# Rita-zi/WavTokenizer

Hardware: AMD Instinct MI355X
Metric: audio-seconds/sec encode+decode, 24 kHz 3 s clips (higher is better)
Workload: dtype f32 (split-f16 x3 products)

## Files before the change

### wavtokenizer_amd/csrc/gemm.hip

```cpp
#include "common.h"
#include <stdlib.h>
#include <cmath>

namespace wt {

typedef float f32x4 __attribute__((ext_vector_type(4)));
typedef float f32x16 __attribute__((ext_vector_type(16)));

static constexpr int BK = 32;
static constexpr int LDS_PITCH = 36;

__device__ __forceinline__ int xcd_remap(int orig, int nwg) {
    int q = nwg >> 3, r = nwg & 7;
    int xcd = orig & 7, idx = orig >> 3;
    int base = xcd < r ? xcd * (q + 1) : r * (q + 1) + (xcd - r) * q;
    return base + idx;
}

__device__ __forceinline__ float elu1(float x) { return x > 0.f ? x : __expf(x) - 1.f; }
__device__ __forceinline__ float gelu_erf(float x) { return x * 0.5f * (1.f + erff(x * 0.70710678118654752440f)); }

template <int BM, int BN, int WAVES_M, int WAVES_N, int PRO, int EPI>
__global__ __launch_bounds__(256) void gemm_kernel(const GemmArgs p) {
    constexpr int WM = BM / WAVES_M, WN = BN / WAVES_N;
// ... 208 lines not shown
                const float bme = in ? p.bias[pc] : 0.f;
                const int f = (pc >> 5) * 16 + (col_l & 15);
#pragma unroll
                for (int r = 0; r < 16; ++r) {
                    const int m = m_w + i * 32 + (r & 3) + 8 * (r >> 2) + row_h;
                    const float mine = acc[i][j][r] + bme;
                    const float ph = __shfl_xor(mine, 16, 64);
                    if (is_mag && in && m < p.M) {
                        float mag = expf(mine);
                        mag = fminf(mag, 100.f);
                        Cg[(long)m * p.c_rstride + f] = mag * cosf(ph);
                        Cg[(long)m * p.c_rstride + p.head_kb + f] = mag * sinf(ph);
                    }
                }
            }
        return;
    }

#pragma unroll
    for (int i = 0; i < TM; ++i)
#pragma unroll
        for (int j = 0; j < TN; ++j) {
            const int n = n_w + j * 32 + col_l;
            if (n >= p.N) continue;
            float bn_ = 0.f, gm = 1.f;
            if (EPI == EPI_BIAS || EPI == EPI_BIAS_RES || EPI == EPI_BIAS_GELU || EPI == EPI_BIAS_GAMMA_RES ||
                EPI == EPI_BIAS_RES_ELU)
                bn_ = p.bias ? p.bias[n] : 0.f;
            if (EPI == EPI_BIAS_GAMMA_RES) gm = p.gamma[n];
#pragma unroll
            for (int r = 0; r < 16; ++r) {
                const int m = m_w + i * 32 + (r & 3) + 8 * (r >> 2) + row_h;
                if (m >= p.M) continue;
                float v = acc[i][j][r];
                if (EPI == EPI_BIAS) {
                    Cg[(long)m * p.c_rstride + n] = v + bn_;
                } else if (EPI == EPI_BIAS_RES) {
                    Cg[(long)m * p.c_rstride + n] = (v + bn_) + p.R[(long)m * p.r_rstride + n];
                } else if (EPI == EPI_BIAS_RES_ELU) {
                    Cg[(long)m * p.c_rstride + n] = elu1((v + bn_) + p.R[(long)m * p.r_rstride + n]);
                } else if (EPI == EPI_BIAS_GELU) {
                    Cg[(long)m * p.c_rstride + n] = gelu_erf(v + bn_);
                } else if (EPI == EPI_BIAS_GAMMA_RES) {
                    Cg[(long)m * p.c_rstride + n] = p.R[(long)m * p.r_rstride + n] + gm * (v + bn_);
                } else if (EPI == EPI_SCALE) {
                    Cg[(long)m * p.c_rstride + n] = v * p.alpha;
                } else if (EPI == EPI_BIAS_ROW) {
// ... 127 lines not shown
```

### wavtokenizer_amd/csrc/gemm16s_kernel.inc

```
template <int BM, int BN, int WAVES_M, int WAVES_N, int NSTAGE, int EPI, int OUT, int DBG = 0, int MF = WT_GEMM16S_MF, int WPS = 2, int KS = 1,
          int PROD = 0>
__global__ __launch_bounds__(64 * WAVES_M * WAVES_N * (1 + PROD), WPS) void G16_NAME(const GemmArgs p G16_PARAMS) {
    constexpr int dbg = DBG;
    static_assert(KS == 1 || (KS == 2 && NSTAGE == 6 && MF == 1 && DBG == 0), "two K tiles per barrier: 6 stages (three pairs), 16x16x32 MFMA, no experiment masks");
    static_assert(!PROD || KS == 2, "loader waves: the two-tiles-per-barrier form only");
    constexpr int NW = WAVES_M * WAVES_N, NT = 64 * NW * (1 + PROD);
    constexpr int NL = PROD ? NW * PROD : NW;
    constexpr int WM = BM / WAVES_M, WN = BN / WAVES_N;
    constexpr int TM = WM / 32, TN = WN / 32;
    constexpr int STG = (BM + BN) * 128;
    constexpr int NPA = BM / 8 / NL, NPB = BN / 8 / NL;
    constexpr int NPT = NPA + NPB;
    static_assert(BM % (8 * NL) == 0 && BN % (8 * NL) == 0, "pieces must divide evenly among the loading waves");
    static_assert(WM % 32 == 0 && WN % 32 == 0 && BM % 16 == 0, "32x32 MFMA tiles");
    static_assert((NSTAGE - 2) * NPT < 64, "vmcnt field");
    extern __shared__ __attribute__((aligned(1024))) char smem_s[];

    const int tid = threadIdx.x, lane = tid & 63;
    const int wave_all = (dbg & 65536) ? (tid >> 6) : __builtin_amdgcn_readfirstlane(tid >> 6);
    const bool loader_wave = PROD && wave_all >= NW;
    const bool mfma_wave = !loader_wave;
    const bool dma_wave = !PROD || loader_wave;
    const int wave = loader_wave ? wave_all - NW : wave_all;
    const int wm = wave / WAVES_N, wn = wave % WAVES_N;
// ... 612 lines not shown
                        }
#pragma unroll
                        for (int it = 0; it < 4; ++it) {
                            const int r = 8 * it + (lane >> 3), ch = lane & 7;
                            const int m = m_w + i * 32 + r;
                            const int n = n0 + 4 * ch;
                            if (m < p.M && (!as_f32 || n < p.N) && !(dbg & 128)) {
                                float* dst = dbase + (long)m * p.c_rstride + n;
                                store_c16<!(dbg & 4096)>(dst, q[it]);
                            }
                        }
                    }
                }
            }
        } else
#pragma unroll
        for (int i = 0; i < TM; ++i) {
#pragma unroll
            for (int j = 0; j < TN; ++j)
#pragma unroll
                for (int g = 0; g < 4; ++g) {
                    const int m = m_w + i * 32 + sub_row(g);
                    const int n = n_w + j * 32 + sub_col(g);
                    if (m >= p.M || n >= p.N) continue;
                    float* crow = Cg + (long)m * p.c_rstride;
                    f32x4 v = acc4(i, j, g);
                    if (EPI == EPI_SCALE || EPI == EPI_BIAS_ROW) {
                        v = EPI == EPI_SCALE ? v * p.alpha : v + p.bias[m];
                        if (n + 3 >= p.N) { if (n + 1 >= p.N) v.y = 0.f; if (n + 2 >= p.N) v.z = 0.f; v.w = 0.f; }
                    }
                    else if (p.bias) v += PCACHE ? *reinterpret_cast<const f32x4*>(pcw + (n - n_w) * 4) : *reinterpret_cast<const f32x4*>(p.bias + n);
                    if (EPI == EPI_BIAS_RES) {
                        v = v + *reinterpret_cast<const f32x4*>(p.R + (long)m * p.r_rstride + n);
                    } else if (EPI == EPI_BIAS_RES_ELU) {
                        v = v + *reinterpret_cast<const f32x4*>(p.R + (long)m * p.r_rstride + n);
                        v.x = elu_s(v.x); v.y = elu_s(v.y); v.z = elu_s(v.z); v.w = elu_s(v.w);
                    } else if (EPI == EPI_BIAS_ELU) {
                        v.x = elu_s(v.x); v.y = elu_s(v.y); v.z = elu_s(v.z); v.w = elu_s(v.w);
                    } else if (EPI == EPI_BIAS_GELU) {
                        v = (dbg & 16384) ? gelu_erf_s4(v) : gelu_erfc_s4(v);
                    } else if (EPI == EPI_BIAS_GAMMA_RES) {
                        const f32x4 gm = *reinterpret_cast<const f32x4*>(pcw + WN * 4 + (n - n_w) * 4);
                        v = *reinterpret_cast<const f32x4*>(p.R + (long)m * p.r_rstride + n) + gm * v;
                    }
                    if (OUT == OUT_S32 || OUT == OUT_S32_DUAL_ELU) store_s32_x4(crow, n, v, amax);
                    else store_c16<(dbg & 262144) != 0>(crow + n, v);
                    if (OUT == OUT_S32_DUAL_ELU) {
// ... 24 lines not shown
```

### wavtokenizer_amd/csrc/ops.hip

```cpp
#include "common.h"
#include <stdlib.h>

namespace wt {

typedef float f32x4 __attribute__((ext_vector_type(4)));

static inline void note_form(int kernel, int variant, int variant2, dim3 grid, unsigned block, size_t lds = 0) {
    if (OpForm* f = g_launch.form) *f = OpForm{kernel, variant, variant2, {grid.x, grid.y, grid.z}, block, (unsigned)lds};
}

__device__ __forceinline__ float wave_sum(float v) {
#pragma unroll
    for (int off = 32; off >= 1; off >>= 1) v += __shfl_xor(v, off, 64);
    return v;
}
typedef _Float16 f16x4s __attribute__((ext_vector_type(4)));
__device__ __forceinline__ void store_s32_1(float* row_base, int e, float v, float& amax) {
    amax = amax1(amax, v);
    _Float16* p = reinterpret_cast<_Float16*>(row_base) + ((e >> 5) * 64 + (e & 31));
    const _Float16 h = (_Float16)v;
    p[0] = h;
    p[32] = (_Float16)((v - (float)h) * 2048.f);
}
__device__ __forceinline__ void store_s32_4(float* row_base, int e, const f32x4 v, float& amax) {
    amax = amax4(amax, v.x, v.y, v.z, v.w);
    f16x4s hi, lo;
    split4_f16(v.x, v.y, v.z, v.w, hi, lo);
    _Float16* p = reinterpret_cast<_Float16*>(row_base) + ((e >> 5) * 64 + (e & 31));
    *reinterpret_cast<f16x4s*>(p) = hi;
    *reinterpret_cast<f16x4s*>(p + 32) = lo;
}
__device__ __forceinline__ float wave_max(float v) {
#pragma unroll
    for (int off = 32; off >= 1; off >>= 1) v = fmaxf(v, __shfl_xor(v, off, 64));
    return v;
}
__device__ __forceinline__ int reflect_pos(int pos, int T, int Tp, bool& ok) {
    if (pos < 0) pos = -pos;
    if (pos >= Tp) pos = 2 * (Tp - 1) - pos;
    ok = pos < T;
    return pos;
}

__global__ __launch_bounds__(256) void conv_first_kernel(const float* __restrict__ wav, const float* __restrict__ w,
                                                         const float* __restrict__ bias, float* __restrict__ y,
                                                         long BT, int T, int k, int Cout, int Tp) {
    const int c4n = Cout >> 2;
    const long total = BT * c4n;
    const int pl = (k - 1) - (k - 1) / 2;
    for (long idx = (long)blockIdx.x * blockDim.x + threadIdx.x; idx < total; idx += (long)gridDim.x * blockDim.x) {
        const long m = idx / c4n;
        const int c = (int)(idx - m * c4n) * 4;
        const long b = m / T;
// ... 110 lines not shown
    const int pl = (k - 1) - (k - 1) / 2, pr = (k - 1) / 2;
    const int maxpad = pl > pr ? pl : pr;
    const int Tp = T > maxpad ? (int)T : maxpad + 1;
    if (Cin == 32 && k == 7 && B <= 65535) {
        note_form(OPK_CONV_LAST32, 0, 0, dim3((unsigned)((T + 255) / 256), B), 256);
        hipLaunchKernelGGL(conv_last32_kernel, dim3((unsigned)((T + 255) / 256), B), dim3(256), 0, s, x, w, bias, y, (int)T, Tp, elu_in);
        WT_HIP_CHECK(hipGetLastError());
        return 0;
    }
    if (Cin < 4 || Cin > 256 || (Cin & (Cin - 1))) { set_error("conv_last: Cin must be a power of two in [4, 256]"); return -1; }
    const long groups = (BT + (256 / (Cin / 4)) - 1) / (256 / (Cin / 4));
    int blocks = (int)(groups < 16384 ? groups : 16384);
    note_form(OPK_CONV_LAST, 0, 0, dim3(blocks), 256);
    hipLaunchKernelGGL(conv_last_kernel, dim3(blocks), dim3(256), 0, s, x, w, bias, y, BT, (int)T, Cin, k, Tp, elu_in);
    WT_HIP_CHECK(hipGetLastError());
    return 0;
}

static constexpr int GN_CH = 128;
__device__ __forceinline__ int mix_len(const int* __restrict__ lens, int b, int Lpad) {
    const int l = lens[b];
    return l < 0 ? 0 : (l > Lpad ? Lpad : l);
}
#define OPS_MIX 0
#define OPS_K(base) base##_kernel
#define OPS_L L
#include "ops_kernel.inc"
#undef OPS_MIX
#undef OPS_K
#undef OPS_L
#define OPS_MIX 1
#define OPS_K(base) base##_mixed_kernel
#define OPS_L Lpad
#include "ops_kernel.inc"
#undef OPS_MIX
#undef OPS_K
#undef OPS_L

int launch_transpose(const float* in, float* out, int B, int R, int C, hipStream_t s, int out_s32, const int* lens) {
    if (out_s32 && (R % 32)) { set_error("transpose: an S32 output needs rows in multiples of 32 elements"); return -1; }
    dim3 grid((C + 31) / 32, (R + 31) / 32, B);
    if (lens) {
        note_form(OPK_TRANSPOSE_MIXED, 0, 0, grid, 256);
        hipLaunchKernelGGL(transpose_mixed_kernel, grid, dim3(256), 0, s, in, out, R, C, out_s32, g_launch.status, lens);
        WT_HIP_CHECK(hipGetLastError());
        return 0;
// ... 37 lines not shown
    const size_t smem = (size_t)GN_CH * GB * cg * sizeof(float);
    if (lens) {
        static PerDeviceOnce attr_mixed;
        if (int rc = attr_mixed.run([&]() -> int { WT_HIP_CHECK(hipFuncSetAttribute(reinterpret_cast<const void*>(gn_chunk_stats_mixed_kernel), hipFuncAttributeMaxDynamicSharedMemorySize, 64 * 1024)); return 0; })) return rc;
        hipLaunchKernelGGL(gn_chunk_stats_mixed_kernel, dim3(groups / GB, nch, B), dim3(256), smem, s, x, part, L, C, cg, GB, groups, nch, lens, lmin);
        const dim3 grid(groups / GB, mode ? nch : 1, B);
        if (mode == 0) hipLaunchKernelGGL(gn_chunk_apply_mixed_kernel<0>, grid, dim3(256), 0, s, x, part, gamma, beta, scale, shift, y, L, C, cg, GB, groups, nch, eps, out_s32, g_launch.status, lens, lmin);
        else if (mode == 1) hipLaunchKernelGGL(gn_chunk_apply_mixed_kernel<1>, grid, dim3(256), 0, s, x, part, gamma, beta, scale, shift, y, L, C, cg, GB, groups, nch, eps, out_s32, g_launch.status, lens, lmin);
        else hipLaunchKernelGGL(gn_chunk_apply_mixed_kernel<2>, grid, dim3(256), 0, s, x, part, gamma, beta, scale, shift, y, L, C, cg, GB, groups, nch, eps, out_s32, g_launch.status, lens, lmin);
        WT_HIP_CHECK(hipGetLastError());
        return 0;
    }
    static PerDeviceOnce attr_once;
    if (int rc = attr_once.run([&]() -> int { WT_HIP_CHECK(hipFuncSetAttribute(reinterpret_cast<const void*>(gn_chunk_stats_kernel), hipFuncAttributeMaxDynamicSharedMemorySize, 64 * 1024)); return 0; })) return rc;
    hipLaunchKernelGGL(gn_chunk_stats_kernel, dim3(groups / GB, nch, B), dim3(256), smem, s, x, part, L, C, cg, GB, groups, nch);
    const dim3 grid(groups / GB, mode ? nch : 1, B);
    note_form(OPK_GN_CHUNK, mode, 0, grid, 256, smem);
    if (mode == 0) hipLaunchKernelGGL(gn_chunk_apply_kernel<0>, grid, dim3(256), 0, s, x, part, gamma, beta, scale, shift, y, L, C, cg, GB, groups, nch, eps, out_s32, g_launch.status);
    else if (mode == 1) hipLaunchKernelGGL(gn_chunk_apply_kernel<1>, grid, dim3(256), 0, s, x, part, gamma, beta, scale, shift, y, L, C, cg, GB, groups, nch, eps, out_s32, g_launch.status);
    else hipLaunchKernelGGL(gn_chunk_apply_kernel<2>, grid, dim3(256), 0, s, x, part, gamma, beta, scale, shift, y, L, C, cg, GB, groups, nch, eps, out_s32, g_launch.status);
    WT_HIP_CHECK(hipGetLastError());
    return 0;
}
static int gn_slab_groups(int C, int groups) {
    const int cg = C / groups;
    for (int g = 1; g <= groups; ++g)
        if (groups % g == 0 && (g * cg) % 32 == 0 && g * cg <= 128) return g;
    return 0;
}

int launch_gn_apply(const float* x, const float* gamma, const float* beta, float* scale, float* shift, float* y,
                    int swish, int B, int L, int C, int groups, float eps, hipStream_t s, int out_s32, float* part, const int* lens) {
    if (out_s32 && (C % 32)) { set_error("gn_apply: an S32 output needs C % 32 == 0"); return -1; }
    const int cg = C / groups;
    int GB = 0;
    for (int g = 1; g <= groups; ++g)
        if (groups % g == 0 && (g * cg) % 32 == 0 && g * cg <= 128) { GB = g; break; }
    if (lens) {
        if (!GB || (cg % 4) || (C % 4) || GB > 8) { set_error("gn_apply: no length-aware form for this channel layout"); return -1; }
        const int lmax = (int)((96 * 1024) / ((size_t)GB * cg * 4));
        if (L > lmax && !part) { set_error("gn_apply: the length-aware launch needs the chunk scratch beyond the slab limit"); return -1; }
        const size_t smem = (size_t)(L < lmax ? L : lmax) * GB * cg * sizeof(float);
        static PerDeviceOnce attr_mixed;
        if (int rc = attr_mixed.run([&]() -> int {
            WT_HIP_CHECK(hipFuncSetAttribute(reinterpret_cast<const void*>(gn_tile_mixed_kernel<0>), hipFuncAttributeMaxDynamicSharedMemorySize, 96 * 1024));
            WT_HIP_CHECK(hipFuncSetAttribute(reinterpret_cast<const void*>(gn_tile_mixed_kernel<1>), hipFuncAttributeMaxDynamicSharedMemorySize, 96 * 1024));
            return 0;
        })) return rc;
        dim3 grid(groups / GB, B);
        const int nt = GB == 4 ? 512 : 256;
        note_form(OPK_GN_MIXED, swish ? 2 : 1, L > lmax ? 3 : 1, grid, nt, smem);
        if (swish) hipLaunchKernelGGL(gn_tile_mixed_kernel<1>, grid, dim3(nt), smem, s, x, gamma, beta, scale, shift, y, L, C, cg, GB, eps, out_s32, g_launch.status, lens, lmax);
        else hipLaunchKernelGGL(gn_tile_mixed_kernel<0>, grid, dim3(nt), smem, s, x, gamma, beta, scale, shift, y, L, C, cg, GB, eps, out_s32, g_launch.status, lens, lmax);
        WT_HIP_CHECK(hipGetLastError());
        if (L > lmax) return launch_gn_chunked(x, gamma, beta, scale, shift, y, swish ? 2 : 1, B, L, C, groups, GB, eps, s, out_s32, part, lens, lmax);
        return 0;
    }
    if (GB && (cg % 4 == 0) && (size_t)L * GB * cg * 4 <= 96 * 1024 && (C % 4 == 0)) {
        const size_t smem = (size_t)L * GB * cg * sizeof(float);
        static PerDeviceOnce attr_once;
        if (int rc = attr_once.run([&]() -> int {
            WT_HIP_CHECK(hipFuncSetAttribute(reinterpret_cast<const void*>(gn_tile_kernel<0>), hipFuncAttributeMaxDynamicSharedMemorySize, 96 * 1024));
            WT_HIP_CHECK(hipFuncSetAttribute(reinterpret_cast<const void*>(gn_tile_kernel<1>), hipFuncAttributeMaxDynamicSharedMemorySize, 96 * 1024));
        return 0;
    })) return rc;
        dim3 grid(groups / GB, B);
        const int nt = GB == 4 ? 512 : 256;
        note_form(OPK_GN_TILE, swish ? 1 : 0, (nt >> 6) == 2 * GB ? 2 : 1, grid, nt, smem);
        if (swish) hipLaunchKernelGGL(gn_tile_kernel<1>, grid, dim3(nt), smem, s, x, gamma, beta, scale, shift, y, L, C, cg, GB, eps, out_s32, g_launch.status);
        else hipLaunchKernelGGL(gn_tile_kernel<0>, grid, dim3(nt), smem, s, x, gamma, beta, scale, shift, y, L, C, cg, GB, eps, out_s32, g_launch.status);
        WT_HIP_CHECK(hipGetLastError());
        return 0;
    }
    if (part && GB && (cg % 4 == 0) && (C % 4 == 0) && GB * cg <= 128 && GB <= 8)
        return launch_gn_chunked(x, gamma, beta, scale, shift, y, swish ? 2 : 1, B, L, C, groups, GB, eps, s, out_s32, part);
    note_form(OPK_GN_STATS, swish ? 2 : 1, 0, dim3(groups, B), 256);
    if (swish)
        hipLaunchKernelGGL(gn_stats_kernel<2>, dim3(groups, B), dim3(256), 0, s, x, gamma, beta, scale, shift, y, L, C,
                           C / groups, eps, out_s32, g_launch.status);
    else
        hipLaunchKernelGGL(gn_stats_kernel<1>, dim3(groups, B), dim3(256), 0, s, x, gamma, beta, scale, shift, y, L, C,
                           C / groups, eps, out_s32, g_launch.status);
    WT_HIP_CHECK(hipGetLastError());
    return 0;
}

template <int NV, int MODE>
__global__ __launch_bounds__(256) void rownorm_kernel(const float* __restrict__ x, float* __restrict__ y, long M, int L,
                                                      const float* __restrict__ dw_w, const float* __restrict__ dw_b,
                                                      const float* __restrict__ in_scale,
                                                      const float* __restrict__ in_shift,
                                                      const float* __restrict__ out_scale,
                                                      const float* __restrict__ out_shift, float eps, int s32, unsigned* status) {
// ... 33 lines not shown
    float sum = 0.f;
#pragma unroll
    for (int i = 0; i < NV; ++i) sum += (v[i].x + v[i].y) + (v[i].z + v[i].w);
    const float mean = wave_sum(sum) * (1.f / C);
    float sq = 0.f;
#pragma unroll
    for (int i = 0; i < NV; ++i) {
        const f32x4 d = v[i] - mean;
        sq += (d.x * d.x + d.y * d.y) + (d.z * d.z + d.w * d.w);
    }
    const float rstd = 1.f / sqrtf(wave_sum(sq) * (1.f / C) + eps);
#pragma unroll
    for (int i = 0; i < NV; ++i) {
        const int c = (i * 64 + lane) * 4;
        const f32x4 os = *reinterpret_cast<const f32x4*>(out_scale + c);
        const f32x4 oh = *reinterpret_cast<const f32x4*>(out_shift + c);
        const f32x4 o = ((v[i] - mean) * rstd) * os + oh;
        if (s32) store_s32_4(y + m * C, c, o, amax);
        else *reinterpret_cast<f32x4*>(y + m * C + c) = o;
    }
    range_report(status, amax);
}

template <int NV>
static int launch_rownorm_nv(int mode, const float* x, float* y, long M, int L, const float* dw_w, const float* dw_b,
                             const float* is, const float* ih, const float* os, const float* oh, float eps,
                             hipStream_t s, int s32, const int* lens) {
    dim3 grid((unsigned)((M + 3) / 4));
    if (mode == RN_DWCONV && lens) {
        const int B = (int)(M / L);
        if (M <= 2048) {
            const long waves = (long)B * L;
            note_form(OPK_DWCONV_LN_MIXED, NV, 1, dim3((unsigned)((waves + 3) / 4)), 256);
            hipLaunchKernelGGL((dwconv_ln_mixed_kernel<NV, 1>), dim3((unsigned)((waves + 3) / 4)), dim3(256), 0, s, x, y, B, L, dw_w, dw_b,
                               os, oh, eps, s32, g_launch.status, lens);
        } else {
            constexpr int R = 4;
            const long waves = (long)B * ((L + R - 1) / R);
            note_form(OPK_DWCONV_LN_MIXED, NV, R, dim3((unsigned)((waves + 3) / 4)), 256);
            hipLaunchKernelGGL((dwconv_ln_mixed_kernel<NV, R>), dim3((unsigned)((waves + 3) / 4)), dim3(256), 0, s, x, y, B, L, dw_w, dw_b,
                               os, oh, eps, s32, g_launch.status, lens);
        }
    }
    else if (mode == RN_DWCONV) {
        const int B = (int)(M / L);
        if (M <= 2048) {
            const long waves = (long)B * L;
            note_form(OPK_DWCONV_LN, NV, 1, dim3((unsigned)((waves + 3) / 4)), 256);
            hipLaunchKernelGGL((dwconv_ln_kernel<NV, 1>), dim3((unsigned)((waves + 3) / 4)), dim3(256), 0, s, x, y, B, L, dw_w, dw_b,
                               os, oh, eps, s32, g_launch.status);
        } else {
            constexpr int R = 4;
            const long waves = (long)B * ((L + R - 1) / R);
            note_form(OPK_DWCONV_LN, NV, R, dim3((unsigned)((waves + 3) / 4)), 256);
            hipLaunchKernelGGL((dwconv_ln_kernel<NV, R>), dim3((unsigned)((waves + 3) / 4)), dim3(256), 0, s, x, y, B, L, dw_w, dw_b,
                               os, oh, eps, s32, g_launch.status);
        }
    }
    else if (mode == RN_PLAIN) {
        note_form(OPK_ROWNORM, NV, RN_PLAIN, grid, 256);
        hipLaunchKernelGGL((rownorm_kernel<NV, RN_PLAIN>), grid, dim3(256), 0, s, x, y, M, L, dw_w, dw_b, is, ih, os, oh, eps, s32, g_launch.status);
    } else {
        note_form(OPK_ROWNORM, NV, RN_AFFINE_IN, grid, 256);
        hipLaunchKernelGGL((rownorm_kernel<NV, RN_AFFINE_IN>), grid, dim3(256), 0, s, x, y, M, L, dw_w, dw_b, is, ih, os, oh, eps, s32, g_launch.status);
    }
    WT_HIP_CHECK(hipGetLastError());
    return 0;
}

int launch_rownorm(int mode, const float* x, float* y, int B, int L, int C, const float* dw_w, const float* dw_b,
                   const float* in_scale, const float* in_shift, const float* out_scale, const float* out_shift,
                   float eps, hipStream_t s, int out_s32, const int* lens) {
    const long M = (long)B * L;
    switch (C) {
        case 256: return launch_rownorm_nv<1>(mode, x, y, M, L, dw_w, dw_b, in_scale, in_shift, out_scale, out_shift, eps, s, out_s32, lens);
        case 512: return launch_rownorm_nv<2>(mode, x, y, M, L, dw_w, dw_b, in_scale, in_shift, out_scale, out_shift, eps, s, out_s32, lens);
        case 768: return launch_rownorm_nv<3>(mode, x, y, M, L, dw_w, dw_b, in_scale, in_shift, out_scale, out_shift, eps, s, out_s32, lens);
        case 1024: return launch_rownorm_nv<4>(mode, x, y, M, L, dw_w, dw_b, in_scale, in_shift, out_scale, out_shift, eps, s, out_s32, lens);
        default: set_error("rownorm: backbone dim must be 256, 512, 768 or 1024"); return -1;
    }
// ... 466 lines not shown
```

### wavtokenizer_amd/csrc/ops_kernel.inc

```

__global__ __launch_bounds__(256) void OPS_K(transpose)(const float* __restrict__ in, float* __restrict__ out, int R,
                                                        int C, int s32, unsigned* status
#if OPS_MIX
                                                        , const int* __restrict__ lens
#endif
                                                        ) {
    __shared__ float tile[32][33];
    float amax = 0.f;
    const long boff = (long)blockIdx.z * R * C;
    const int c0 = blockIdx.x * 32, r0 = blockIdx.y * 32;
    const int tx = threadIdx.x & 31, ty = threadIdx.x >> 5;
    for (int i = ty; i < 32; i += 8) {
        const int r = r0 + i, c = c0 + tx;
        if (r < R && c < C) tile[i][tx] = in[boff + (long)r * C + c];
    }
    __syncthreads();
    for (int i = ty; i < 32; i += 8) {
        const int c = c0 + i, r = r0 + tx;
        if (r < R && c < C) {
#if OPS_MIX
            const float v = c < mix_len(lens, blockIdx.z, C) ? tile[tx][i] : 0.f;
            if (s32) store_s32_1(out + boff + (long)c * R, r, v, amax);
            else out[boff + (long)c * R + r] = v;
#else
// ... 49 lines not shown
    if (threadIdx.x == 0) s_rstd = 1.f / sqrtf((red[0] + red[1] + red[2] + red[3]) / (float)n + eps);
    __syncthreads();
    if (threadIdx.x < cg) {
        const int c = g * cg + threadIdx.x;
        const float sc = s_rstd * gamma[c];
        scale[(long)b * C + c] = sc;
        shift[(long)b * C + c] = beta[c] - mean * sc;
    }
    if (APPLY) {
        float* yb = y + (long)b * OPS_L * C + g * cg;
        const float rstd = s_rstd;
        for (int i = threadIdx.x; i < n; i += 256) {
            const int t = i / cg, j = i - t * cg;
            const float sc = rstd * gamma[g * cg + j];
            float v = xb[(long)t * C + j] * sc + (beta[g * cg + j] - mean * sc);
            if (APPLY == 2) v = v / (1.f + expf(-v));
            if (s32) store_s32_1(y + ((long)b * OPS_L + t) * C, g * cg + j, v, amax);
            else yb[(long)t * C + j] = v;
        }
        range_report(status, amax);
    }
}

template <int SWISH>
__global__ __launch_bounds__(512) void OPS_K(gn_tile)(const float* __restrict__ x, const float* __restrict__ gamma,
                                                      const float* __restrict__ beta, float* __restrict__ scale,
                                                      float* __restrict__ shift, float* __restrict__ y, int OPS_L, int C,
                                                      int cg, int GB, float eps, int s32, unsigned* status
#if OPS_MIX
                                                      , const int* __restrict__ lens, int lmax
#endif
                                                      ) {
    extern __shared__ __attribute__((aligned(16))) float tile[];
    float amax = 0.f;
    __shared__ float s_sc[128], s_sh[128], s_red[8];
    const int NT = blockDim.x;
    const int W = GB * cg, W4 = W / 4;
    const int c0 = blockIdx.x * W, b = blockIdx.y;
#if OPS_MIX
    const int L = mix_len(lens, b, Lpad);
    if (L > lmax) return;
#endif
    const float* xb = x + (long)b * OPS_L * C + c0;
    const int dt = NT / W4, dq = NT - dt * W4;
    {
        int t = threadIdx.x / W4, q = threadIdx.x - t * W4;
        for (; t < L; t += dt, q += dq) {
// ... 65 lines not shown
        }
    }
    __syncthreads();
    float* yb = y + (long)b * OPS_L * C;
#if OPS_MIX
    for (int e = threadIdx.x; e < (Lpad - L) * W4; e += NT) {
        const int tz = e / W4, q = e - tz * W4;
        const f32x4 z = {0.f, 0.f, 0.f, 0.f};
        if (s32) store_s32_4(yb + (long)(L + tz) * C, c0 + q * 4, z, amax);
        else *reinterpret_cast<f32x4*>(yb + (long)(L + tz) * C + c0 + q * 4) = z;
    }
#endif
    {
        int t = threadIdx.x / W4, q = threadIdx.x - t * W4;
        for (; t < L; t += dt, q += dq) {
            if (q >= W4) { q -= W4; ++t; if (t >= L) break; }
            const f32x4 v = *reinterpret_cast<const f32x4*>(tile + t * W + q * 4);
            const f32x4 sc = *reinterpret_cast<const f32x4*>(s_sc + q * 4), sh = *reinterpret_cast<const f32x4*>(s_sh + q * 4);
            f32x4 o = v * sc + sh;
            if (SWISH) {
                o.x *= __builtin_amdgcn_rcpf(1.f + __expf(-o.x)); o.y *= __builtin_amdgcn_rcpf(1.f + __expf(-o.y));
                o.z *= __builtin_amdgcn_rcpf(1.f + __expf(-o.z)); o.w *= __builtin_amdgcn_rcpf(1.f + __expf(-o.w));
            }
            if (s32) store_s32_4(yb + (long)t * C, c0 + q * 4, o, amax);
            else *reinterpret_cast<f32x4*>(yb + (long)t * C + c0 + q * 4) = o;
        }
    }
    range_report(status, amax);
}


__global__ __launch_bounds__(256) void OPS_K(gn_chunk_stats)(const float* __restrict__ x, float* __restrict__ part, int OPS_L,
                                                             int C, int cg, int GB, int groups, int nch
#if OPS_MIX
                                                             , const int* __restrict__ lens, int lmin
#endif
                                                             ) {
    extern __shared__ __attribute__((aligned(16))) float tile[];
    const int W = GB * cg, W4 = W / 4;
    const int c0 = blockIdx.x * W, k = blockIdx.y, b = blockIdx.z;
#if OPS_MIX
    const int L = mix_len(lens, b, Lpad);
    if (L <= lmin || k * GN_CH >= L) return;
#endif
    const int t0 = k * GN_CH, rows = L - t0 < GN_CH ? L - t0 : GN_CH;
    const float* xb = x + ((long)b * OPS_L + t0) * C + c0;
    for (int e = threadIdx.x; e < rows * W4; e += 256) {
        const int t = e / W4, q = e - t * W4;
// ... 80 lines not shown
        f32x4 o = v * sc + sh;
        if (APPLY == 2) {
            o.x *= __builtin_amdgcn_rcpf(1.f + __expf(-o.x)); o.y *= __builtin_amdgcn_rcpf(1.f + __expf(-o.y));
            o.z *= __builtin_amdgcn_rcpf(1.f + __expf(-o.z)); o.w *= __builtin_amdgcn_rcpf(1.f + __expf(-o.w));
        }
        if (s32) store_s32_4(yb + (long)t * C, c0 + q * 4, o, amax);
        else *reinterpret_cast<f32x4*>(yb + (long)t * C + c0 + q * 4) = o;
    }
#if OPS_MIX
    {
        const int rz0 = rows > 0 ? rows : 0, rz1 = Lpad - t0 < GN_CH ? Lpad - t0 : GN_CH;
        const f32x4 z = {0.f, 0.f, 0.f, 0.f};
        for (int e = threadIdx.x + rz0 * W4; e < rz1 * W4; e += 256) {
            const int t = e / W4, q = e - t * W4;
            if (s32) store_s32_4(yb + (long)t * C, c0 + q * 4, z, amax);
            else *reinterpret_cast<f32x4*>(yb + (long)t * C + c0 + q * 4) = z;
        }
    }
#endif
#undef OPS_NCH
    range_report(status, amax);
}

template <int NV, int R>
__global__ __launch_bounds__(256) void OPS_K(dwconv_ln)(const float* __restrict__ x, float* __restrict__ y, int B, int OPS_L,
                                                        const float* __restrict__ dw_w, const float* __restrict__ dw_b,
                                                        const float* __restrict__ out_scale,
                                                        const float* __restrict__ out_shift, float eps, int s32, unsigned* status
#if OPS_MIX
                                                        , const int* __restrict__ lens
#endif
                                                        ) {
    constexpr int C = NV * 256;
    const int lane = threadIdx.x & 63;
    float amax = 0.f;
    const int per_clip = (OPS_L + R - 1) / R;
    const long wq = (long)blockIdx.x * 4 + (threadIdx.x >> 6);
    if (wq >= (long)B * per_clip) return;
    const int b = (int)(wq / per_clip);
    const int t0 = (int)(wq - (long)b * per_clip) * R;
#if OPS_MIX
    const int L = mix_len(lens, b, Lpad);
#endif
    const float* xb = x + (long)b * OPS_L * C;
    f32x4 v[R][NV];
#pragma unroll
    for (int i = 0; i < NV; ++i) {
        const int c = (i * 64 + lane) * 4;
        f32x4 xr[R + 6], w[7];
#pragma unroll
        for (int k = 0; k < R + 6; ++k) {
            const int tt = t0 + k - 3;
            xr[k] = (tt >= 0 && tt < L) ? *reinterpret_cast<const f32x4*>(xb + (long)tt * C + c) : (f32x4){0.f, 0.f, 0.f, 0.f};
        }
#pragma unroll
        for (int j = 0; j < 7; ++j) w[j] = *reinterpret_cast<const f32x4*>(dw_w + j * C + c);
        const f32x4 bias = *reinterpret_cast<const f32x4*>(dw_b + c);
#pragma unroll
        for (int r = 0; r < R; ++r) {
            f32x4 acc = bias;
#pragma unroll
            for (int j = 0; j < 7; ++j) {
                const int tt = t0 + r + j - 3;
                if (tt >= 0 && tt < L) acc += xr[r + j] * w[j];
            }
            v[r][i] = acc;
        }
    }
#pragma unroll
    for (int r = 0; r < R; ++r) {
#if OPS_MIX
        if (t0 + r >= Lpad) break;
        if (t0 + r >= L) {
            float* zrow = y + ((long)b * Lpad + t0 + r) * C;
            const f32x4 z = {0.f, 0.f, 0.f, 0.f};
#pragma unroll
            for (int i = 0; i < NV; ++i) {
                const int c = (i * 64 + lane) * 4;
                if (s32) store_s32_4(zrow, c, z, amax);
                else *reinterpret_cast<f32x4*>(zrow + c) = z;
            }
            continue;
        }
#else
        if (t0 + r >= L) break;
#endif
        float sum = 0.f;
#pragma unroll
        for (int i = 0; i < NV; ++i) sum += (v[r][i].x + v[r][i].y) + (v[r][i].z + v[r][i].w);
        const float mean = wave_sum(sum) * (1.f / C);
        float sq = 0.f;
#pragma unroll
        for (int i = 0; i < NV; ++i) {
            const f32x4 d = v[r][i] - mean;
            sq += (d.x * d.x + d.y * d.y) + (d.z * d.z + d.w * d.w);
        }
        const float rstd = 1.f / sqrtf(wave_sum(sq) * (1.f / C) + eps);
        float* yrow = y + ((long)b * OPS_L + t0 + r) * C;
#pragma unroll
        for (int i = 0; i < NV; ++i) {
            const int c = (i * 64 + lane) * 4;
            const f32x4 os = *reinterpret_cast<const f32x4*>(out_scale + c);
            const f32x4 oh = *reinterpret_cast<const f32x4*>(out_shift + c);
            const f32x4 o = ((v[r][i] - mean) * rstd) * os + oh;
            if (s32) store_s32_4(yrow, c, o, amax);
            else *reinterpret_cast<f32x4*>(yrow + c) = o;
        }
    }
    range_report(status, amax);
}

__global__ __launch_bounds__(256) void OPS_K(softmax)(float* __restrict__ S, long rows, int OPS_L, int ld, float* __restrict__ P_s32
#if OPS_MIX
                                                      , const int* __restrict__ lens
#endif
                                                      ) {
    const int lane = threadIdx.x & 63;
    const long r = (long)blockIdx.x * 4 + (threadIdx.x >> 6);
    if (r >= rows) return;
#if OPS_MIX
    const int L = mix_len(lens, (int)(r / Lpad), Lpad);
#endif
    float* row = S + r * ld;
    float mx = -INFINITY;
    for (int j = lane; j < L; j += 64) mx = fmaxf(mx, row[j]);
    mx = wave_max(mx);
    float sum = 0.f;
    for (int j0 = 4 * lane; j0 < L; j0 += 256)
        for (int j = j0; j < j0 + 4 && j < L; ++j) {
            const float e = expf(row[j] - mx);
// ... 105 lines not shown
```

### wavtokenizer_amd/csrc/plan.cpp

```cpp
#include "model.h"

namespace wt {

static bool site_fp32(const wt_plan* P, int site) { return (P->fp32_sites >> site) & 1u; }
static bool plan_fp32(const wt_plan* P) {
    if ((P->flags & WT_PLAN_FLAG_FP32_GEMM) || !P->model->s32_ok) return true;
    if (P->whole_site == SITE_SEADEC && !P->model->sd_s32_ok) return true;
    return P->whole_site >= 0 && site_fp32(P, P->whole_site);
}
static bool plan_unfused(const wt_plan* P) { return P->flags & WT_PLAN_FLAG_UNFUSED; }
static bool plan_s32(const wt_plan* P) { return !plan_unfused(P) && !plan_fp32(P); }

static int gemm_auto(const wt_plan* P, const GemmArgs& a, int pro, int epi, hipStream_t s) {
    if (P->model->f32_stale.load()) if (int rc = ensure_f32_weights(P->model)) return rc;
    return launch_gemm(a, pro, epi, s);
}

static void set_s32(GemmArgs& a, const S32Copy& c) {
    a.W_hi = c.p; a.acc_scale = c.acc_scale; a.tap_pair = c.tap_pair ? 1 : 0;
}

static int gemm_s32(const GemmArgs& a, int epi, int out, hipStream_t s, const int* mix = nullptr) {
    if (!a.W_hi) { set_error("internal: no S32 copy of this weight"); return WT_ERR_INVALID; }
    return launch_gemm16s(a, epi, out, s, mix);
// ... 401 lines not shown
        }, 1, "res.gn2");
        GemmArgs a2 = zconv_args(r.c2, B, L);
        a2.r_rstride = D;
        gemm_step(P, s32, a2, in_place(h1, x), PRO_NONE, EPI_BIAS_RES, OUT_F32, "res.conv2");
        snapshot(x, name);
    };
    resnet(M->res[0], "bb.pos_net.0", SITE_RES0);
    resnet(M->res[1], "bb.pos_net.1", SITE_RES1);
    {
        P->cur_site = SITE_ATTN;
        const bool s32 = s32_at(SITE_ATTN) && M->at_Wqk.s32.p && M->at_Wv.s32.p && M->at_Wp.s32.p;
        const int fmt = s32 ? BUF_S32 : BUF_F32;
        P->bufs[h1].fmt = fmt;
        const int qk = P->buf("bb.attn.qk", (size_t)Mrows * 2 * D, fmt);
        const int vt = P->buf("bb.attn.vt", (size_t)B * D * Lp, fmt);
        const int S = P->buf("bb.attn.s", (size_t)Mrows * Lp);
        const int Ps = s32 ? P->buf("bb.attn.p", (size_t)Mrows * Lp, BUF_S32) : S;
        const int o = P->buf("bb.attn.o", (size_t)Mrows * D, fmt);
        P->step({x, sc, sh, gp, h1}, [=](const RunCtx& c) {
            return launch_gn_apply(P->ptr(c, x), M->at_nw, M->at_nb, P->ptr(c, sc), P->ptr(c, sh), P->ptr(c, h1), 0, B, L, D, 32, 1e-6f, c.stream, s32, P->ptr(c, gp), lens(c));
        }, 1, "attn.gn");
        gemm_step(P, s32, linear_args(M->at_Wqk, M->at_bqk, Mrows, 2 * D, D), {h1, -1, qk}, PRO_NONE, EPI_BIAS, OUT_S32, "attn.qk");
        P->step({h1, vt}, [=](const RunCtx& c) {
            if (int rc = launch_fill_u32(P->ptr(c, vt), 0u, (size_t)B * D * Lp * sizeof(float), c.stream)) return rc;
            GemmArgs a = linear_args(nullptr, M->at_bv, D, L, D);
            a.A = s32 ? static_cast<const float*>(M->at_Wv.s32.p) : M->at_Wv.w; a.acc_scale = M->at_Wv.s32.acc_scale; a.zA = 0;
            a.zW = (long)L * D; a.nz = B;
            a.C = P->ptr(c, vt); a.c_rstride = Lp; a.zC = (long)D * Lp;
            return dense_act(P, s32, a, P->ptr(c, h1), EPI_BIAS_ROW, OUT_S32, c.stream);
        }, 2, "attn.vt");
        P->step({qk, S}, [=](const RunCtx& c) {
            GemmArgs a = linear_args(nullptr, nullptr, L, L, D);
            a.A = P->ptr(c, qk); a.a_rstride = 2 * D; a.zA = (long)L * 2 * D;
            a.w_rstride = 2 * D; a.zW = (long)L * 2 * D; a.nz = B;
            a.C = P->ptr(c, S); a.c_rstride = Lp; a.zC = (long)L * Lp;
            a.alpha = (float)std::pow((double)D, -0.5);
            return dense_act(P, s32, a, P->ptr(c, qk) + D, EPI_SCALE, OUT_F32, c.stream);
        }, 1, "attn.s");
        P->step({S, Ps}, [=](const RunCtx& c) { return launch_softmax(P->ptr(c, S), (int)Mrows, L, Lp, c.stream, s32 ? P->ptr(c, Ps) : nullptr, lens(c)); });
        P->step({Ps, vt, o}, [=](const RunCtx& c) {
            GemmArgs a = linear_args(nullptr, nullptr, L, D, Lp);
            a.A = P->ptr(c, Ps); a.zA = (long)L * Lp;
            a.zW = (long)D * Lp; a.nz = B;
            a.C = P->ptr(c, o); a.c_rstride = D; a.zC = (long)L * D;
            return dense_act(P, s32, a, P->ptr(c, vt), EPI_BIAS, OUT_S32, c.stream);
        }, 1, "attn.o");
        GemmArgs ap = linear_args(M->at_Wp, M->at_bp, Mrows, D, D);
        ap.r_rstride = D;
        gemm_step(P, s32, ap, in_place(o, x), PRO_NONE, EPI_BIAS_RES, OUT_F32, "attn.proj");
        snapshot(x, "bb.pos_net.2");
    }
    resnet(M->res[2], "bb.pos_net.3", SITE_RES2);
    resnet(M->res[3], "bb.pos_net.4", SITE_RES3);
// ... 167 lines not shown
```

Before: 39560.

## Zero V^T padding inside GEMM epilogue and template dwconv-LN/GN kernels on form flags

```diff
diff --git a/wavtokenizer_amd/csrc/gemm.hip b/wavtokenizer_amd/csrc/gemm.hip
--- a/wavtokenizer_amd/csrc/gemm.hip
+++ b/wavtokenizer_amd/csrc/gemm.hip
@@ -254,7 +254,16 @@
 #pragma unroll
         for (int j = 0; j < TN; ++j) {
             const int n = n_w + j * 32 + col_l;
-            if (n >= p.N) continue;
+            if (n >= p.N) {
+                if (EPI == EPI_BIAS_ROW && n < p.c_rstride && p.c_rstride == ((p.N + 31) & ~31)) {
+#pragma unroll
+                    for (int r = 0; r < 16; ++r) {
+                        const int m = m_w + i * 32 + (r & 3) + 8 * (r >> 2) + row_h;
+                        if (m < p.M) Cg[(long)m * p.c_rstride + n] = 0.f;
+                    }
+                }
+                continue;
+            }
             float bn_ = 0.f, gm = 1.f;
             if (EPI == EPI_BIAS || EPI == EPI_BIAS_RES || EPI == EPI_BIAS_GELU || EPI == EPI_BIAS_GAMMA_RES ||
                 EPI == EPI_BIAS_RES_ELU)
diff --git a/wavtokenizer_amd/csrc/gemm16s_kernel.inc b/wavtokenizer_amd/csrc/gemm16s_kernel.inc
--- a/wavtokenizer_amd/csrc/gemm16s_kernel.inc
+++ b/wavtokenizer_amd/csrc/gemm16s_kernel.inc
@@ -658,7 +658,12 @@
                 for (int g = 0; g < 4; ++g) {
                     const int m = m_w + i * 32 + sub_row(g);
                     const int n = n_w + j * 32 + sub_col(g);
-                    if (m >= p.M || n >= p.N) continue;
+                    if (m >= p.M) continue;
+                    if (n >= p.N) {
+                        if (EPI == EPI_BIAS_ROW && n < p.c_rstride && p.c_rstride == ((p.N + 31) & ~31))
+                            store_s32_x4(Cg + (long)m * p.c_rstride, n, (f32x4){0.f, 0.f, 0.f, 0.f}, amax);
+                        continue;
+                    }
                     float* crow = Cg + (long)m * p.c_rstride;
                     f32x4 v = acc4(i, j, g);
                     if (EPI == EPI_SCALE || EPI == EPI_BIAS_ROW) {
diff --git a/wavtokenizer_amd/csrc/ops.hip b/wavtokenizer_amd/csrc/ops.hip
--- a/wavtokenizer_amd/csrc/ops.hip
+++ b/wavtokenizer_amd/csrc/ops.hip
@@ -29,6 +29,21 @@
     _Float16* p = reinterpret_cast<_Float16*>(row_base) + ((e >> 5) * 64 + (e & 31));
     *reinterpret_cast<f16x4s*>(p) = hi;
     *reinterpret_cast<f16x4s*>(p + 32) = lo;
+}
+__device__ __forceinline__ void store_s32_4_pair(float* row_base, int e, const f32x4 v, float& amax) {
+    typedef unsigned u32x2s __attribute__((ext_vector_type(2)));
+    typedef unsigned u32x4s __attribute__((ext_vector_type(4)));
+    amax = amax4(amax, v.x, v.y, v.z, v.w);
+    f16x4s hi, lo;
+    split4_f16(v.x, v.y, v.z, v.w, hi, lo);
+    const u32x2s h = __builtin_bit_cast(u32x2s, hi), l = __builtin_bit_cast(u32x2s, lo);
+    const bool odd = (e >> 2) & 1;
+    const unsigned s0 = odd ? h.x : l.x, s1 = odd ? h.y : l.y;
+    const unsigned r0 = (unsigned)__builtin_amdgcn_update_dpp(0, (int)s0, 0xB1, 0xF, 0xF, true);
+    const unsigned r1 = (unsigned)__builtin_amdgcn_update_dpp(0, (int)s1, 0xB1, 0xF, 0xF, true);
+    const u32x4s o = odd ? (u32x4s){r0, r1, l.x, l.y} : (u32x4s){h.x, h.y, r0, r1};
+    _Float16* p = reinterpret_cast<_Float16*>(row_base) + ((e >> 5) * 64 + (odd ? 32 + (e & 31) - 4 : (e & 31)));
+    *reinterpret_cast<u32x4s*>(p) = o;
 }
 __device__ __forceinline__ float wave_max(float v) {
 #pragma unroll
@@ -185,6 +200,7 @@
     const int l = lens[b];
     return l < 0 ? 0 : (l > Lpad ? Lpad : l);
 }
+enum : int { DWLN_PAIR = 1, DWLN_LDS = 2, DWLN_ILV = 4 };
 #define OPS_MIX 0
 #define OPS_K(base) base##_kernel
 #define OPS_L L
@@ -268,6 +284,7 @@
     WT_HIP_CHECK(hipGetLastError());
     return 0;
 }
+constexpr int GN_PAIR = 0;
 static int gn_slab_groups(int C, int groups) {
     const int cg = C / groups;
     for (int g = 1; g <= groups; ++g)
@@ -289,15 +306,15 @@
         const size_t smem = (size_t)(L < lmax ? L : lmax) * GB * cg * sizeof(float);
         static PerDeviceOnce attr_mixed;
         if (int rc = attr_mixed.run([&]() -> int {
-            WT_HIP_CHECK(hipFuncSetAttribute(reinterpret_cast<const void*>(gn_tile_mixed_kernel<0>), hipFuncAttributeMaxDynamicSharedMemorySize, 96 * 1024));
-            WT_HIP_CHECK(hipFuncSetAttribute(reinterpret_cast<const void*>(gn_tile_mixed_kernel<1>), hipFuncAttributeMaxDynamicSharedMemorySize, 96 * 1024));
+            WT_HIP_CHECK(hipFuncSetAttribute(reinterpret_cast<const void*>(gn_tile_mixed_kernel<0, GN_PAIR>), hipFuncAttributeMaxDynamicSharedMemorySize, 96 * 1024));
+            WT_HIP_CHECK(hipFuncSetAttribute(reinterpret_cast<const void*>(gn_tile_mixed_kernel<1, GN_PAIR>), hipFuncAttributeMaxDynamicSharedMemorySize, 96 * 1024));
             return 0;
         })) return rc;
         dim3 grid(groups / GB, B);
         const int nt = GB == 4 ? 512 : 256;
         note_form(OPK_GN_MIXED, swish ? 2 : 1, L > lmax ? 3 : 1, grid, nt, smem);
-        if (swish) hipLaunchKernelGGL(gn_tile_mixed_kernel<1>, grid, dim3(nt), smem, s, x, gamma, beta, scale, shift, y, L, C, cg, GB, eps, out_s32, g_launch.status, lens, lmax);
-        else hipLaunchKernelGGL(gn_tile_mixed_kernel<0>, grid, dim3(nt), smem, s, x, gamma, beta, scale, shift, y, L, C, cg, GB, eps, out_s32, g_launch.status, lens, lmax);
+        if (swish) hipLaunchKernelGGL((gn_tile_mixed_kernel<1, GN_PAIR>), grid, dim3(nt), smem, s, x, gamma, beta, scale, shift, y, L, C, cg, GB, eps, out_s32, g_launch.status, lens, lmax);
+        else hipLaunchKernelGGL((gn_tile_mixed_kernel<0, GN_PAIR>), grid, dim3(nt), smem, s, x, gamma, beta, scale, shift, y, L, C, cg, GB, eps, out_s32, g_launch.status, lens, lmax);
         WT_HIP_CHECK(hipGetLastError());
         if (L > lmax) return launch_gn_chunked(x, gamma, beta, scale, shift, y, swish ? 2 : 1, B, L, C, groups, GB, eps, s, out_s32, part, lens, lmax);
         return 0;
@@ -306,15 +323,15 @@
         const size_t smem = (size_t)L * GB * cg * sizeof(float);
         static PerDeviceOnce attr_once;
         if (int rc = attr_once.run([&]() -> int {
-            WT_HIP_CHECK(hipFuncSetAttribute(reinterpret_cast<const void*>(gn_tile_kernel<0>), hipFuncAttributeMaxDynamicSharedMemorySize, 96 * 1024));
-            WT_HIP_CHECK(hipFuncSetAttribute(reinterpret_cast<const void*>(gn_tile_kernel<1>), hipFuncAttributeMaxDynamicSharedMemorySize, 96 * 1024));
+            WT_HIP_CHECK(hipFuncSetAttribute(reinterpret_cast<const void*>(gn_tile_kernel<0, GN_PAIR>), hipFuncAttributeMaxDynamicSharedMemorySize, 96 * 1024));
+            WT_HIP_CHECK(hipFuncSetAttribute(reinterpret_cast<const void*>(gn_tile_kernel<1, GN_PAIR>), hipFuncAttributeMaxDynamicSharedMemorySize, 96 * 1024));
         return 0;
     })) return rc;
         dim3 grid(groups / GB, B);
         const int nt = GB == 4 ? 512 : 256;
         note_form(OPK_GN_TILE, swish ? 1 : 0, (nt >> 6) == 2 * GB ? 2 : 1, grid, nt, smem);
-        if (swish) hipLaunchKernelGGL(gn_tile_kernel<1>, grid, dim3(nt), smem, s, x, gamma, beta, scale, shift, y, L, C, cg, GB, eps, out_s32, g_launch.status);
-        else hipLaunchKernelGGL(gn_tile_kernel<0>, grid, dim3(nt), smem, s, x, gamma, beta, scale, shift, y, L, C, cg, GB, eps, out_s32, g_launch.status);
+        if (swish) hipLaunchKernelGGL((gn_tile_kernel<1, GN_PAIR>), grid, dim3(nt), smem, s, x, gamma, beta, scale, shift, y, L, C, cg, GB, eps, out_s32, g_launch.status);
+        else hipLaunchKernelGGL((gn_tile_kernel<0, GN_PAIR>), grid, dim3(nt), smem, s, x, gamma, beta, scale, shift, y, L, C, cg, GB, eps, out_s32, g_launch.status);
         WT_HIP_CHECK(hipGetLastError());
         return 0;
     }
@@ -394,40 +411,36 @@
     range_report(status, amax);
 }
 
+template <int NV, int R, int FORM, int WPB>
+static int launch_dwconv_ln_form(const float* x, float* y, int B, int L, const float* dw_w, const float* dw_b, const float* os,
+                                 const float* oh, float eps, int s32, const int* lens, int max_blocks, hipStream_t s) {
+    const long waves = (long)B * ((L + R - 1) / R);
+    long blocks = (waves + WPB - 1) / WPB;
+    if ((FORM & DWLN_LDS) && max_blocks > 0 && blocks > max_blocks) blocks = max_blocks;
+    const dim3 grid((unsigned)blocks);
+    note_form(lens ? OPK_DWCONV_LN_MIXED : OPK_DWCONV_LN, NV, R, grid, WPB * 64);
+    if (lens)
+        hipLaunchKernelGGL((dwconv_ln_mixed_kernel<NV, R, FORM, WPB>), grid, dim3(WPB * 64), 0, s, x, y, B, L, dw_w, dw_b, os, oh, eps,
+                           s32, g_launch.status, lens);
+    else
+        hipLaunchKernelGGL((dwconv_ln_kernel<NV, R, FORM, WPB>), grid, dim3(WPB * 64), 0, s, x, y, B, L, dw_w, dw_b, os, oh, eps,
+                           s32, g_launch.status);
+    WT_HIP_CHECK(hipGetLastError());
+    return 0;
+}
+constexpr int DWLN_SMALL_FORM = 0, DWLN_LARGE_FORM = 0, DWLN_LARGE_WPB = 4;
+
 template <int NV>
 static int launch_rownorm_nv(int mode, const float* x, float* y, long M, int L, const float* dw_w, const float* dw_b,
                              const float* is, const float* ih, const float* os, const float* oh, float eps,
                              hipStream_t s, int s32, const int* lens) {
     dim3 grid((unsigned)((M + 3) / 4));
-    if (mode == RN_DWCONV && lens) {
+    if (mode == RN_DWCONV) {
         const int B = (int)(M / L);
-        if (M <= 2048) {
-            const long waves = (long)B * L;
-            note_form(OPK_DWCONV_LN_MIXED, NV, 1, dim3((unsigned)((waves + 3) / 4)), 256);
-            hipLaunchKernelGGL((dwconv_ln_mixed_kernel<NV, 1>), dim3((unsigned)((waves + 3) / 4)), dim3(256), 0, s, x, y, B, L, dw_w, dw_b,
-                               os, oh, eps, s32, g_launch.status, lens);
-        } else {
-            constexpr int R = 4;
-            const long waves = (long)B * ((L + R - 1) / R);
-            note_form(OPK_DWCONV_LN_MIXED, NV, R, dim3((unsigned)((waves + 3) / 4)), 256);
-            hipLaunchKernelGGL((dwconv_ln_mixed_kernel<NV, R>), dim3((unsigned)((waves + 3) / 4)), dim3(256), 0, s, x, y, B, L, dw_w, dw_b,
-                               os, oh, eps, s32, g_launch.status, lens);
-        }
-    }
-    else if (mode == RN_DWCONV) {
-        const int B = (int)(M / L);
-        if (M <= 2048) {
-            const long waves = (long)B * L;
-            note_form(OPK_DWCONV_LN, NV, 1, dim3((unsigned)((waves + 3) / 4)), 256);
-            hipLaunchKernelGGL((dwconv_ln_kernel<NV, 1>), dim3((unsigned)((waves + 3) / 4)), dim3(256), 0, s, x, y, B, L, dw_w, dw_b,
-                               os, oh, eps, s32, g_launch.status);
-        } else {
-            constexpr int R = 4;
-            const long waves = (long)B * ((L + R - 1) / R);
-            note_form(OPK_DWCONV_LN, NV, R, dim3((unsigned)((waves + 3) / 4)), 256);
-            hipLaunchKernelGGL((dwconv_ln_kernel<NV, R>), dim3((unsigned)((waves + 3) / 4)), dim3(256), 0, s, x, y, B, L, dw_w, dw_b,
-                               os, oh, eps, s32, g_launch.status);
-        }
+        int rc;
+        if (M <= 2048) rc = launch_dwconv_ln_form<NV, 1, DWLN_SMALL_FORM, 4>(x, y, B, L, dw_w, dw_b, os, oh, eps, s32, lens, 0, s);
+        else rc = launch_dwconv_ln_form<NV, 4, DWLN_LARGE_FORM, DWLN_LARGE_WPB>(x, y, B, L, dw_w, dw_b, os, oh, eps, s32, lens, 0, s);
+        if (rc) return rc;
     }
     else if (mode == RN_PLAIN) {
         note_form(OPK_ROWNORM, NV, RN_PLAIN, grid, 256);
diff --git a/wavtokenizer_amd/csrc/ops_kernel.inc b/wavtokenizer_amd/csrc/ops_kernel.inc
--- a/wavtokenizer_amd/csrc/ops_kernel.inc
+++ b/wavtokenizer_amd/csrc/ops_kernel.inc
@@ -95,7 +95,7 @@
     }
 }
 
-template <int SWISH>
+template <int SWISH, int PAIR>
 __global__ __launch_bounds__(512) void OPS_K(gn_tile)(const float* __restrict__ x, const float* __restrict__ gamma,
                                                       const float* __restrict__ beta, float* __restrict__ scale,
                                                       float* __restrict__ shift, float* __restrict__ y, int OPS_L, int C,
@@ -207,8 +207,9 @@
                 o.x *= __builtin_amdgcn_rcpf(1.f + __expf(-o.x)); o.y *= __builtin_amdgcn_rcpf(1.f + __expf(-o.y));
                 o.z *= __builtin_amdgcn_rcpf(1.f + __expf(-o.z)); o.w *= __builtin_amdgcn_rcpf(1.f + __expf(-o.w));
             }
-            if (s32) store_s32_4(yb + (long)t * C, c0 + q * 4, o, amax);
-            else *reinterpret_cast<f32x4*>(yb + (long)t * C + c0 + q * 4) = o;
+            if (!s32) *reinterpret_cast<f32x4*>(yb + (long)t * C + c0 + q * 4) = o;
+            else if (PAIR) store_s32_4_pair(yb + (long)t * C, c0 + q * 4, o, amax);
+            else store_s32_4(yb + (long)t * C, c0 + q * 4, o, amax);
         }
     }
     range_report(status, amax);
@@ -335,8 +336,8 @@
     range_report(status, amax);
 }
 
-template <int NV, int R>
-__global__ __launch_bounds__(256) void OPS_K(dwconv_ln)(const float* __restrict__ x, float* __restrict__ y, int B, int OPS_L,
+template <int NV, int R, int FORM, int WPB>
+__global__ __launch_bounds__(WPB * 64) void OPS_K(dwconv_ln)(const float* __restrict__ x, float* __restrict__ y, int B, int OPS_L,
                                                         const float* __restrict__ dw_w, const float* __restrict__ dw_b,
                                                         const float* __restrict__ out_scale,
                                                         const float* __restrict__ out_shift, float eps, int s32, unsigned* status
@@ -344,12 +345,25 @@
                                                         , const int* __restrict__ lens
 #endif
                                                         ) {
-    constexpr int C = NV * 256;
+    constexpr int C = NV * 256, C4 = C / 4;
+    constexpr bool PAIR = (FORM & DWLN_PAIR) != 0, PLDS = (FORM & DWLN_LDS) != 0, ILV = (FORM & DWLN_ILV) != 0;
+    __shared__ __attribute__((aligned(16))) float s_par[PLDS ? 10 * C : 4];
     const int lane = threadIdx.x & 63;
     float amax = 0.f;
     const int per_clip = (OPS_L + R - 1) / R;
-    const long wq = (long)blockIdx.x * 4 + (threadIdx.x >> 6);
-    if (wq >= (long)B * per_clip) return;
+    const long total = (long)B * per_clip;
+    if (PLDS) {
+        for (int e = threadIdx.x; e < 10 * C4; e += WPB * 64) {
+            const int row = e / C4, q = e - row * C4;
+            const float* src = row < 7 ? dw_w + row * C : row == 7 ? dw_b : row == 8 ? out_scale : out_shift;
+            *reinterpret_cast<f32x4*>(s_par + row * C + q * 4) = *reinterpret_cast<const f32x4*>(src + q * 4);
+        }
+        __syncthreads();
+    }
+    auto par = [&](int row, const float* g, int c) -> f32x4 {
+        return PLDS ? *reinterpret_cast<const f32x4*>(s_par + row * C + c) : *reinterpret_cast<const f32x4*>(g + c);
+    };
+    for (long wq = (long)blockIdx.x * WPB + (threadIdx.x >> 6); wq < total; wq += PLDS ? (long)gridDim.x * WPB : total) {
     const int b = (int)(wq / per_clip);
     const int t0 = (int)(wq - (long)b * per_clip) * R;
 #if OPS_MIX
@@ -367,8 +381,8 @@
             xr[k] = (tt >= 0 && tt < L) ? *reinterpret_cast<const f32x4*>(xb + (long)tt * C + c) : (f32x4){0.f, 0.f, 0.f, 0.f};
         }
 #pragma unroll
-        for (int j = 0; j < 7; ++j) w[j] = *reinterpret_cast<const f32x4*>(dw_w + j * C + c);
-        const f32x4 bias = *reinterpret_cast<const f32x4*>(dw_b + c);
+        for (int j = 0; j < 7; ++j) w[j] = par(j, dw_w + j * C, c);
+        const f32x4 bias = par(7, dw_b, c);
 #pragma unroll
         for (int r = 0; r < R; ++r) {
             f32x4 acc = bias;
@@ -379,6 +393,36 @@
             }
             v[r][i] = acc;
         }
+    }
+    float mean[R], rstd[R];
+    if (ILV) {
+        float sum[R], sq[R];
+#pragma unroll
+        for (int r = 0; r < R; ++r) {
+            sum[r] = 0.f;
+#pragma unroll
+            for (int i = 0; i < NV; ++i) sum[r] += (v[r][i].x + v[r][i].y) + (v[r][i].z + v[r][i].w);
+        }
+#pragma unroll
+        for (int off = 32; off >= 1; off >>= 1)
+#pragma unroll
+            for (int r = 0; r < R; ++r) sum[r] += __shfl_xor(sum[r], off, 64);
+#pragma unroll
+        for (int r = 0; r < R; ++r) {
+            mean[r] = sum[r] * (1.f / C);
+            sq[r] = 0.f;
+#pragma unroll
+            for (int i = 0; i < NV; ++i) {
+                const f32x4 d = v[r][i] - mean[r];
+                sq[r] += (d.x * d.x + d.y * d.y) + (d.z * d.z + d.w * d.w);
+            }
+        }
+#pragma unroll
+        for (int off = 32; off >= 1; off >>= 1)
+#pragma unroll
+            for (int r = 0; r < R; ++r) sq[r] += __shfl_xor(sq[r], off, 64);
+#pragma unroll
+        for (int r = 0; r < R; ++r) rstd[r] = 1.f / sqrtf(sq[r] * (1.f / C) + eps);
     }
 #pragma unroll
     for (int r = 0; r < R; ++r) {
@@ -398,27 +442,31 @@
 #else
         if (t0 + r >= L) break;
 #endif
-        float sum = 0.f;
-#pragma unroll
-        for (int i = 0; i < NV; ++i) sum += (v[r][i].x + v[r][i].y) + (v[r][i].z + v[r][i].w);
-        const float mean = wave_sum(sum) * (1.f / C);
-        float sq = 0.f;
-#pragma unroll
-        for (int i = 0; i < NV; ++i) {
-            const f32x4 d = v[r][i] - mean;
-            sq += (d.x * d.x + d.y * d.y) + (d.z * d.z + d.w * d.w);
-        }
-        const float rstd = 1.f / sqrtf(wave_sum(sq) * (1.f / C) + eps);
+        if (!ILV) {
+            float sum = 0.f;
+#pragma unroll
+            for (int i = 0; i < NV; ++i) sum += (v[r][i].x + v[r][i].y) + (v[r][i].z + v[r][i].w);
+            mean[r] = wave_sum(sum) * (1.f / C);
+            float sq = 0.f;
+#pragma unroll
+            for (int i = 0; i < NV; ++i) {
+                const f32x4 d = v[r][i] - mean[r];
+                sq += (d.x * d.x + d.y * d.y) + (d.z * d.z + d.w * d.w);
+            }
+            rstd[r] = 1.f / sqrtf(wave_sum(sq) * (1.f / C) + eps);
+        }
         float* yrow = y + ((long)b * OPS_L + t0 + r) * C;
 #pragma unroll
         for (int i = 0; i < NV; ++i) {
             const int c = (i * 64 + lane) * 4;
-            const f32x4 os = *reinterpret_cast<const f32x4*>(out_scale + c);
-            const f32x4 oh = *reinterpret_cast<const f32x4*>(out_shift + c);
-            const f32x4 o = ((v[r][i] - mean) * rstd) * os + oh;
-            if (s32) store_s32_4(yrow, c, o, amax);
-            else *reinterpret_cast<f32x4*>(yrow + c) = o;
-        }
+            const f32x4 os = par(8, out_scale, c);
+            const f32x4 oh = par(9, out_shift, c);
+            const f32x4 o = ((v[r][i] - mean[r]) * rstd[r]) * os + oh;
+            if (!s32) *reinterpret_cast<f32x4*>(yrow + c) = o;
+            else if (PAIR) store_s32_4_pair(yrow, c, o, amax);
+            else store_s32_4(yrow, c, o, amax);
+        }
+    }
     }
     range_report(status, amax);
 }
diff --git a/wavtokenizer_amd/csrc/plan.cpp b/wavtokenizer_amd/csrc/plan.cpp
--- a/wavtokenizer_amd/csrc/plan.cpp
+++ b/wavtokenizer_amd/csrc/plan.cpp
@@ -447,13 +447,12 @@
         }, 1, "attn.gn");
         gemm_step(P, s32, linear_args(M->at_Wqk, M->at_bqk, Mrows, 2 * D, D), {h1, -1, qk}, PRO_NONE, EPI_BIAS, OUT_S32, "attn.qk");
         P->step({h1, vt}, [=](const RunCtx& c) {
-            if (int rc = launch_fill_u32(P->ptr(c, vt), 0u, (size_t)B * D * Lp * sizeof(float), c.stream)) return rc;
             GemmArgs a = linear_args(nullptr, M->at_bv, D, L, D);
             a.A = s32 ? static_cast<const float*>(M->at_Wv.s32.p) : M->at_Wv.w; a.acc_scale = M->at_Wv.s32.acc_scale; a.zA = 0;
             a.zW = (long)L * D; a.nz = B;
             a.C = P->ptr(c, vt); a.c_rstride = Lp; a.zC = (long)D * Lp;
             return dense_act(P, s32, a, P->ptr(c, h1), EPI_BIAS_ROW, OUT_S32, c.stream);
-        }, 2, "attn.vt");
+        }, 1, "attn.vt");
         P->step({qk, S}, [=](const RunCtx& c) {
             GemmArgs a = linear_args(nullptr, nullptr, L, L, D);
             a.A = P->ptr(c, qk); a.a_rstride = 2 * D; a.zA = (long)L * 2 * D;
```

Result: no change. 39360 (-0.5%).
